# cure-lab/MotionCraft

Measured on AMD Instinct MI355X. Metric: sampled SMPL-X frames/sec (196-frame seq, 1000-step DDPM), higher is better.
Workload: dtype f32

## Files before the change

### include/motioncraft_amd.h

```cpp
#ifndef MOTIONCRAFT_AMD_H
#define MOTIONCRAFT_AMD_H
#include <stdint.h>

#ifdef __cplusplus
extern "C" {
#endif

#define MC_OK 0
#define MC_ERR_ARG 1
#define MC_ERR_HIP 2
#define MC_ERR_STATE 3

typedef struct mc_model mc_model;
typedef struct mc_ctx mc_ctx;

typedef struct mc_model_config {
    int32_t input_feats;
    int32_t max_seq_len;
    int32_t latent_dim;
    int32_t num_parts;
    int32_t num_layers;
    int32_t ffn_dim;
    int32_t time_embed_dim;
    int32_t text_latent_dim;
// ... 78 lines not shown

int mc_ctx_graph_capture(mc_ctx* c, float* x_dev, const float* noise_dev, const mc_step_coefs* coefs_host, int32_t num_steps,
                         void* stream);
int mc_ctx_graph_step(mc_ctx* c, int32_t step_index, void* stream);
int mc_ctx_graph_release(mc_ctx* c);

int mc_sample_step_seeded(mc_ctx* c, float* x_t_dev, int32_t step_index, const mc_step_coefs* coefs,
                          const float* noise_dev, const mc_seed* seed, float* x_prev_dev, float* x0_dev, void* stream);

int mc_sample_step_inpaint(mc_ctx* c, const float* x_t_dev, int32_t step_index, const mc_step_coefs* coefs,
                           const float* noise_dev, const mc_inpaint* inpaint, float* x_prev_dev, float* x0_dev,
                           void* stream);

int mc_ctx_get_buffer(mc_ctx* c, const char* name, int32_t layer, void** dev_ptr, int64_t* numel);

int mc_debug_flop_ledger(int32_t enable);
int64_t mc_debug_flop_ledger_dump(char* buf, int64_t cap);

int mc_op_gemm(const float* a_dev, const float* w_dev, const float* bias_dev, const float* res_dev,
               float* c_dev, int32_t M, int32_t N, int32_t K, int32_t ldw, int32_t act, void* stream);
int mc_op_gemm_f16(const float* a_dev, const float* w_dev, const float* bias_dev, const float* res_dev, float* c_dev,
                   int32_t M, int32_t N, int32_t K, int32_t split, void* stream);
int mc_op_gemm_f16_planes(const void* a_hi_dev, const void* a_lo_dev, const float* w_dev, const float* bias_dev, const float* res_dev,
                          float* c_dev, int32_t M, int32_t N, int32_t K, int32_t split, int32_t pre, int32_t frag_major, void* stream);
int mc_op_gemm_tail(const float* h_dev, const float* a_dev, const float* w_dev, const float* bias_dev, float* c_dev, float* c2_dev,
                    int32_t M, int32_t N, int32_t K, float wc, float wu, int32_t variant, void* stream);
int mc_op_ln_rows(const float* x_dev, int64_t ldx, const float* gamma_dev, const float* beta_dev,
                  const float* add_dev, int32_t add_mod, float* y_dev, int64_t rows, int32_t L, void* stream);
enum { MC_TEMPORAL_STEP = 0,
       MC_TEMPORAL_WHOLE = 1,
       MC_TEMPORAL_LSPLIT = 2,
       MC_TEMPORAL_PAIR = 3,
       MC_TEMPORAL_F16X3 = 4,
       MC_TEMPORAL_F16 = 5 };
int mc_op_body_attention(const float* mf_dev, int64_t ldmf, const float* qkv_dev, const float* wsm_dev, float* ys_dev, int64_t frames,
                         int32_t H, int32_t L, int64_t twin_from, const int32_t* split_flag_dev, int64_t frame0, void* stream);
int mc_op_temporal_attention(const float* mf_dev, const float* tf_dev, const float* mask_dev, float* yt_dev, int32_t b0, int32_t nb,
                             int32_t B, int32_t T, int32_t Nt, int32_t H, int32_t L, int32_t form, int32_t skip_text,
                             const int32_t* twin_flag_dev, void* stream);
enum { MC_ENC_ATTN_LAYER = 0,
       MC_ENC_ATTN_SMALL = 1,
       MC_ENC_ATTN_STREAM = 2 };
int mc_op_enc_ln(const float* x_dev, const float* gamma_dev, const float* beta_dev, float* y_dev, int64_t rows, int32_t L, float eps,
                 int32_t relu, void* stream);
int mc_op_enc_embed_tokens(const int32_t* ids_dev, const float* emb_dev, const float* pos_dev, float* x_dev, int64_t rows, int32_t S,
                           int32_t d, int32_t vocab, void* stream);
int mc_op_enc_attention(const float* qkv_dev, const uint8_t* valid_dev, float* out_dev, int32_t B, int32_t S, int32_t d, int32_t heads,
                        int32_t causal, int32_t form, void* stream);
typedef struct mc_gemm_strided {
    const float* a_dev; int64_t lda, a_gstride;
    const float* w_dev; int64_t ldw, w_gstride;
    const float* bias_dev; int64_t b_gstride;
    float* c_dev; int64_t ldc, c_gstride;
    const float* res_dev; int64_t ldr, r_gstride;
    const float* add_dev; int64_t ld_add, dup_rows;
    int32_t add_mod, act, act_after_res, M, N, K;
} mc_gemm_strided;
int mc_op_gemm_strided(int32_t mode, int32_t groups, const mc_gemm_strided* args, void* stream);
int mc_op_bigru_steps(const float* gi_dev, const float* whh_dev, const float* bhh_dev, float* h_dev, const int32_t* lens_dev,
                      int32_t len_div, int32_t B, int32_t S, int32_t H, int32_t s0, int32_t steps, void* stream);
int mc_op_conv1d_k4s2(const float* x_dev, int64_t ldx, const float* w_tapmajor_dev, const float* bias_dev, float* y_padded_dev, int32_t B,
                      int32_t T, int32_t C, int32_t Cp, int32_t O, float slope, void* stream);
int mc_op_sampler_update(const float* x_t_dev, const float* out_text_dev, const float* out_none_dev,
                         const float* noise_dev, float* x_prev_dev, float* x0_dev, int64_t n,
                         const mc_step_coefs* coefs, void* stream);

#define MC_POST_MAXTAP 129
// ... 187 lines not shown
```

### motioncraft_amd/csrc/mc_attn.hip

```cpp
#include "mc_common.h"
#include "mc_kernels.h"
#include <utility>
#include <stdlib.h>

namespace {

template <int HD, int H>
__global__ __launch_bounds__(256) void body_reg_k(const float* __restrict__ mf, long ldmf, const float* __restrict__ qkv,
                                                   const float* __restrict__ wsm, float* __restrict__ ys, long frames,
                                                   TwinAlias alias, long frame0) {
    constexpr int G = 8, L = G * HD;
    constexpr int GPW = 64 / HD;
    __shared__ float s_w[H * H];
    for (int i = threadIdx.x; i < H * H; i += 256) s_w[i] = wsm[i];
    __syncthreads();
    const int lane = threadIdx.x & 63;
    const long wave = (long)blockIdx.x * 4 + (threadIdx.x >> 6);
    const long grp = wave * GPW + lane / HD;
    const long frame = grp / G;
    const int gh = (int)(grp % G), l = lane % HD;
    if (frame >= frames) return;
    if (alias.split_flag && frame0 + frame >= alias.from && *alias.split_flag == 0) return;
    const int c = gh * HD + l;
    const long tok0 = frame * H;
// ... 35 lines not shown
        static_for_16(contract_kv);
#pragma unroll
        for (int h = 0; h < H; ++h) {
            float st = 0.f;
#pragma unroll
            for (int j = 0; j < H; ++j) st += s_w[h * H + j] * bv[j];
            float dy = 0.f;
            auto contract_qa = [&](auto S) { dy += row_ror<decltype(S)::value>(q[h]) * A_[decltype(S)::value]; };
            static_for_16(contract_qa);
            out[h * L] = st + (bv[h] + dy);
        }
    } else {
        float A[HD];
#pragma unroll
        for (int d = 0; d < HD; ++d) {
            float a = 0.f;
#pragma unroll
            for (int h = 0; h < H; ++h) a += __shfl(k[h], d, HD) * v[h];
            A[d] = a;
        }
#pragma unroll
        for (int h = 0; h < H; ++h) {
            float st = 0.f;
#pragma unroll
            for (int j = 0; j < H; ++j) st += s_w[h * H + j] * bv[j];
            float dy = 0.f;
#pragma unroll
            for (int d = 0; d < HD; ++d) dy += __shfl(q[h], d, HD) * A[d];
            out[h * L] = st + (bv[h] + dy);
        }
    }
}

template <int L, bool LSPLIT, bool PAIR = false>
__global__ __launch_bounds__(256, 3) void temporal_k(const float* __restrict__ mf, const float* __restrict__ tf,
                                                     const float* __restrict__ mask, float* __restrict__ yt,
                                                     int b0, int B, int T, int Nt, int H, const int* twin_flag, int skip_text) {
    static_assert(!PAIR || (L == 64 && !LSPLIT), "temporal_k: PAIR is the L = 64 whole-part form");
    constexpr int LW = PAIR ? 2 * L : L;
    constexpr int NT = L / 32;
    constexpr int LP = LW + 4;
    constexpr int C4 = LW / 4;
    constexpr int NSL = 256 / C4;
    constexpr int NACC = LSPLIT ? 1 : NT;
    __shared__ __attribute__((aligned(16))) float sm[2 * LW + 2 * NSL * LW + 2 * 32 * LP + (LSPLIT ? NT * 32 * 33 : 0)];
    float* s_m = sm;
    float* s_s = s_m + LW;
    float* s_pm = s_s + LW;
    float* s_ps = s_pm + NSL * LW;
    float* Ks = s_ps + NSL * LW;
    float* Vs = Ks + 32 * LP;
    float* Qs = Ks;
    float* Ps = Vs + 32 * LP;
    const int ls = LSPLIT ? (int)blockIdx.y : 0;

    const int tid = threadIdx.x, lane = tid & 63, wave = tid >> 6;
    const int HB = PAIR ? H / 2 : H;
    const int b = b0 + blockIdx.x / HB, h = PAIR ? 2 * (blockIdx.x % HB) : blockIdx.x % HB;
    const int wp = PAIR ? wave >> 1 : 0, wl = PAIR ? wave & 1 : wave;
    const float cnd = b < B ? 1.f : 0.f;
    const int bm = (twin_flag && b >= B && *twin_flag == 0) ? b - B : b;
    const float* mrow = mask + (long)(b % B) * T;
    const int Nseq = Nt + T;
    const float NEG = -1000000.f;
    const long D4 = 4 * L;
    const int hf = lane >> 5;

    auto row_ptr = [&](int n, int c4, int& t) -> const float* {
        const int nc = n < Nseq ? n : Nseq - 1;
        const bool txt = nc < Nt;
        t = txt ? 0 : nc - Nt;
        const int pp = PAIR ? c4 / L : 0, cc = PAIR ? c4 % L : c4;
        const float* rt = tf + ((long)b * Nt + (txt ? nc : 0)) * 2 * L + cc;
        const float* rm = mf + (((long)bm * T + t) * H + h + pp) * D4 + L + cc;
        return txt ? rt : rm;
    };
    auto issue_kv = [&](int n, int c4, f32x4& kk, f32x4& vv, float& mv) {
        int t;
        const float* r = row_ptr(n, c4, t);
        kk = *reinterpret_cast<const f32x4*>(r);
        vv = *reinterpret_cast<const f32x4*>(r + L);
        const float mm = mrow[t];
        mv = n < Nt ? cnd : mm;
    };
    auto issue_k = [&](int n, int c4, f32x4& kk, float& mv) {
        int t;
        const float* r = row_ptr(n, c4, t);
        kk = *reinterpret_cast<const f32x4*>(r);
        const float mm = mrow[t];
        mv = n < Nt ? cnd : mm;
    };

    constexpr int BATCH = LSPLIT ? 12 : 8;
    int skip1 = 0, skip2 = 0;
    if constexpr (!LSPLIT) {
        if (b >= B && skip_text) {
            int v = 0;
            for (int t = tid; t < T; t += 256) v |= mrow[t] != 0.f;
            if (__syncthreads_or(v)) { skip1 = Nt / (NSL * BATCH) * (NSL * BATCH); skip2 = Nt / 32 * 32; }
        }
    }

    {
        const int c4 = (tid % C4) * 4, sl = tid / C4;
        f32x4 m = {-3e38f, -3e38f, -3e38f, -3e38f}, s = {0.f, 0.f, 0.f, 0.f};
        for (int n0 = skip1 + sl; n0 < Nseq; n0 += NSL * BATCH) {
            f32x4 kk[BATCH];
            float mv[BATCH];
#pragma unroll
            for (int u = 0; u < BATCH; ++u) issue_k(n0 + u * NSL, c4, kk[u], mv[u]);
#pragma unroll
            for (int u = 0; u < BATCH; ++u) {
                const bool ok = n0 + u * NSL < Nseq;
                const float add = (1.f - mv[u]) * NEG;
#pragma unroll
                for (int j = 0; j < 4; ++j) kk[u][j] = ok ? (kk[u][j] + add) * LOG2E : -3e38f;
            }
#pragma unroll
            for (int j = 0; j < 4; ++j) {
                float nm = m[j];
#pragma unroll
                for (int u = 0; u < BATCH; ++u) nm = fmaxf(nm, kk[u][j]);
                float acc = s[j] * fast_exp2(m[j] - nm);
#pragma unroll
                for (int u = 0; u < BATCH; ++u) acc += fast_exp2(kk[u][j] - nm);
                s[j] = acc;
                m[j] = nm;
            }
        }
        *reinterpret_cast<f32x4*>(s_pm + sl * LW + c4) = m;
        *reinterpret_cast<f32x4*>(s_ps + sl * LW + c4) = s;
    }
    __syncthreads();
    if (tid < LW) {
        float M = -3e38f;
        for (int i = 0; i < NSL; ++i) M = fmaxf(M, s_pm[i * LW + tid]);
        float S = 0.f;
        for (int i = 0; i < NSL; ++i) S += s_ps[i * LW + tid] * fast_exp2(s_pm[i * LW + tid] - M);
        s_m[tid] = M;
        s_s[tid] = 1.f / S;
    }
    __syncthreads();

    const bool mm_active = PAIR || wave < NT;
    f32x16 acc[NACC];
#pragma unroll
    for (int dt = 0; dt < NACC; ++dt)
#pragma unroll
        for (int r = 0; r < 16; ++r) acc[dt][r] = 0.f;
    const int nch = (Nseq + 31) / 32;
    constexpr int SPT = (32 * C4) / 256;
    f32x4 pk[SPT], pv[SPT];
    float pm[SPT];
    auto prefetch_kv = [&](int ch) {
#pragma unroll
        for (int j = 0; j < SPT; ++j) {
            const int i = tid + 256 * j;
            issue_kv(ch * 32 + i / C4, (i % C4) * 4, pk[j], pv[j], pm[j]);
        }
    };
    const int ch0 = skip2 / 32;
    prefetch_kv(ch0);
    for (int ch = ch0; ch < nch; ++ch) {
#pragma unroll
        for (int j = 0; j < SPT; ++j) {
            const int i = tid + 256 * j;
            const int row = i / C4, c4 = (i % C4) * 4;
            const int n = ch * 32 + row;
            f32x4 e = {0.f, 0.f, 0.f, 0.f}, v = {0.f, 0.f, 0.f, 0.f};
            if (n < Nseq) {
                const float add = (1.f - pm[j]) * NEG;
#pragma unroll
                for (int q = 0; q < 4; ++q) {
                    e[q] = fast_exp2(fmaf(pk[j][q] + add, LOG2E, -s_m[c4 + q])) * s_s[c4 + q];
                    v[q] = pv[j][q] * pm[j];
                }
            }
            *reinterpret_cast<f32x4*>(Ks + row * LP + c4) = e;
            *reinterpret_cast<f32x4*>(Vs + row * LP + c4) = v;
        }
        __syncthreads();
        if (ch + 1 < nch) prefetch_kv(ch + 1);
        __builtin_amdgcn_sched_barrier(0);
        if (mm_active) {
#pragma unroll 4
            for (int ks = 0; ks < 16; ++ks) {
                const int n = 2 * ks + hf;
                if constexpr (LSPLIT) {
                    const float bb = Vs[n * LP + ls * 32 + (lane & 31)];
                    const float a = Ks[n * LP + wave * 32 + (lane & 31)];
                    acc[0] = __builtin_amdgcn_mfma_f32_32x32x2f32(a, bb, acc[0], 0, 0, 0);
                } else {
                    const float bb = Vs[n * LP + wp * L + wl * 32 + (lane & 31)];
#pragma unroll
                    for (int dt = 0; dt < NT; ++dt) {
                        const float a = Ks[n * LP + wp * L + dt * 32 + (lane & 31)];
                        acc[dt] = __builtin_amdgcn_mfma_f32_32x32x2f32(a, bb, acc[dt], 0, 0, 0);
                    }
                }
            }
        }
        __syncthreads();
    }

    const int ntc = (T + 31) / 32;
    constexpr int SEG = LW / 8;
    constexpr int QG = PAIR ? 4 : 8;
    const int qrow = tid >> 3, qsub = tid & 7;
    const int qpart = PAIR ? qsub >> 2 : 0, qcol = PAIR ? (qsub & 3) * SEG : qsub * SEG;
    float qv[SEG];
    auto prefetch_q = [&](int tc) {
        const int t = tc * 32 + qrow;
        if (t < T) {
            const float* r = mf + (((long)bm * T + t) * H + h + qpart) * D4 + 3 * L + qcol;
#pragma unroll
            for (int j = 0; j < SEG; j += 4) {
                const f32x4 x = *reinterpret_cast<const f32x4*>(r + j);
                qv[j] = x[0]; qv[j + 1] = x[1]; qv[j + 2] = x[2]; qv[j + 3] = x[3];
            }
        }
    };
    const int tc0 = LSPLIT ? (int)blockIdx.z : 0, tcs = LSPLIT ? (int)gridDim.z : 1;
    prefetch_q(tc0);
    for (int tc = tc0; tc < ntc; tc += tcs) {
        {
            const int t = tc * 32 + qrow;
            float mx = -3e38f;
            if (t < T) {
#pragma unroll
                for (int j = 0; j < SEG; ++j) mx = fmaxf(mx, qv[j]);
            }
            mx = group_max(mx, QG);
            float s = 0.f;
            if (t < T) {
#pragma unroll
// ... 46 lines not shown
            for (int i = tid; i < 32 * 32; i += 256) {
                const int tr = i >> 5, l = i & 31, t = tc * 32 + tr;
                float v = Ps[tr * 33 + l];
#pragma unroll
                for (int w = 1; w < NT; ++w) v += Ps[(w * 32 + tr) * 33 + l];
                if (t < T) yt[((long)b * T + t) * (H * L) + h * L + ls * 32 + l] = v;
            }
        }
    }
}

}

int mc_launch_body(const float* mf, long ldmf, const float* qkv, const float* wsm, float* ys,
                   long frames, int H, int L, int G, hipStream_t s, TwinAlias alias, long frame0) {
    MC_REQUIRE(G == 8 && (H == 12 || H == 8) && (L == 32 || L == 64 || L == 128), "body: H=%d L=%d G=%d unsupported", H, L, G);
    if (frames <= 0) return MC_OK;
    const int hd = L / G;
    const long groups = frames * G;
    const long waves = (groups * hd + 63) / 64;
    dim3 grid((unsigned)((waves + 3) / 4));
    MC_LEDGER("body_reg_k", grid, (double)frames * (2.0 * H * H * L + G * 2.0 * (2.0 * H * hd * hd)));
#define MC_BODY_CASE(HH)                                                                                          \
    if (hd == 16) hipLaunchKernelGGL((body_reg_k<16, HH>), grid, dim3(256), 0, s, mf, ldmf, qkv, wsm, ys, frames, alias, frame0);    \
    else if (hd == 8) hipLaunchKernelGGL((body_reg_k<8, HH>), grid, dim3(256), 0, s, mf, ldmf, qkv, wsm, ys, frames, alias, frame0); \
    else hipLaunchKernelGGL((body_reg_k<4, HH>), grid, dim3(256), 0, s, mf, ldmf, qkv, wsm, ys, frames, alias, frame0);
    if (H == 12) { MC_BODY_CASE(12) } else { MC_BODY_CASE(8) }
#undef MC_BODY_CASE
    MC_LAUNCH_CHECK();
    return MC_OK;
}

int mc_launch_temporal(const float* mf, const float* tf, const float* mask, float* yt,
                       int b0, int nb, int B, int T, int Nt, int H, int L, hipStream_t s, const int* twin_flag, long lsplit_max, bool pair, bool skip_text) {
    const int sk = skip_text ? 1 : 0;
    if (nb <= 0) return MC_OK;
    dim3 grid(nb * H), blk(256);
    if (mc_ledger_on) {
        char name[32];
        snprintf(name, sizeof(name), "temporal_k<%d", L);
        dim3 lg = grid;
        if (L >= 64 && (long)nb * H <= lsplit_max) { lg.y = L / 32; lg.z = (long)nb * H * (L / 32) * 2 <= 256 ? 2 : 1; }
        else if (L == 64 && pair && H % 2 == 0) lg.x = nb * (H / 2);
        MC_LEDGER(name, lg, (double)nb * H * (2.0 * (Nt + T) * L * L + 2.0 * T * L * L));
    }
    if (L >= 64 && (long)nb * H <= lsplit_max) {
        grid.y = L / 32;
        grid.z = (long)nb * H * (L / 32) * 2 <= 256 ? 2 : 1;
        if (L == 128) hipLaunchKernelGGL((temporal_k<128, true>), grid, blk, 0, s, mf, tf, mask, yt, b0, B, T, Nt, H, twin_flag, sk);
        else hipLaunchKernelGGL((temporal_k<64, true>), grid, blk, 0, s, mf, tf, mask, yt, b0, B, T, Nt, H, twin_flag, sk);
        MC_LAUNCH_CHECK();
        return MC_OK;
    }
    if (L == 128) hipLaunchKernelGGL((temporal_k<128, false>), grid, blk, 0, s, mf, tf, mask, yt, b0, B, T, Nt, H, twin_flag, sk);
    else if (L == 64 && pair && H % 2 == 0) {
        grid.x = nb * (H / 2);
        hipLaunchKernelGGL((temporal_k<64, false, true>), grid, blk, 0, s, mf, tf, mask, yt, b0, B, T, Nt, H, twin_flag, sk);
    } else if (L == 64) hipLaunchKernelGGL((temporal_k<64, false>), grid, blk, 0, s, mf, tf, mask, yt, b0, B, T, Nt, H, twin_flag, sk);
    else if (L == 32) hipLaunchKernelGGL((temporal_k<32, false>), grid, blk, 0, s, mf, tf, mask, yt, b0, B, T, Nt, H, twin_flag, sk);
    else { mc_set_error("temporal: latent_dim=%d unsupported (32, 64, 128)", L); return MC_ERR_ARG; }
    MC_LAUNCH_CHECK();
    return MC_OK;
}
```

### motioncraft_amd/csrc/mc_kernels.h

```cpp
#pragma once
#include <hip/hip_runtime.h>
#include <stdint.h>
#include "mc_options.h"

struct TwinAlias {
    const int* split_flag = nullptr;
    long from = 0;
};

int mc_launch_ln_rows(const float* X, long ldx, int x_col, const float* gamma, const float* beta,
                      const float* add, int add_mod, float* Y, long ldy, long rows, int L, hipStream_t s);
struct StepRef {
    const int* ptr = nullptr;
    long stride = 0;
};
int mc_launch_film_rows(const float* Y1, const float* Y2, const float* gamma, const float* beta,
                        const float* ss, float* A, long rows, int D, hipStream_t s, TwinAlias y1_alias = TwinAlias(), long row0 = 0,
                        StepRef step = StepRef(), int y1_parts = 1, long y1_pstride = 0,
                        int planes = 0, long plane_stride = 0);
int mc_launch_timestep_embedding(const int* t_orig, float* te, int S, int D, hipStream_t s);
int mc_launch_silu(const float* X, float* Y, long n, hipStream_t s);
int mc_launch_add_rows(float* out, const float* a, const float* b, const float* bias, long rows, int D, hipStream_t s);
int mc_launch_softmax_rows_small(const float* W, float* out, int rows, int cols, hipStream_t s);

// ... 56 lines not shown
    int* idx;
    float* gate;
    uint32_t* key;
    float* comb_w;
    int* src_row;
    int* dst_row;
    int* tile_group; int* tile_row0; int* tile_nrows;
    int* state;
    int max_tiles;
    uint32_t tie_xor = 0xFFFFFFFFu;
};
size_t mc_route_state_ints(int E);
bool mc_route_is_small(const McOptions& o, long N);
bool mc_route_cleans_counts(const McOptions& o, long N);
size_t mc_route_barrier_offset();
size_t mc_route_error_offset();
int mc_route_coop_wgs(long N);
int mc_route_coop_slots(int dev);
bool mc_route_coop_reserve(int dev, int nwg);
void mc_route_coop_release(int dev, int nwg);
size_t mc_route_barrier_ints();
int mc_launch_gate_finish(const float* proj, const float* sim_n, const float* logit_scale, long N, int E,
                          RouteBufs rb, hipStream_t s);
int mc_launch_route(long N, long Nsrc, long gsplit, int E, int capacity, RouteBufs rb, const McOptions& o, hipStream_t s);
const int* mc_route_num_tiles_ptr(const RouteBufs& rb, int group = 0);
const int* mc_route_split_flag_ptr(const RouteBufs& rb);

int mc_launch_body(const float* mf, long ldmf, const float* qkv, const float* wsm, float* ys,
                   long frames, int H, int L, int G, hipStream_t s, TwinAlias alias = TwinAlias(), long frame0 = 0);
int mc_launch_temporal(const float* mf, const float* tf, const float* mask, float* yt,
                       int b0, int nb, int B, int T, int Nt, int H, int L, hipStream_t s, const int* twin_flag = nullptr,
                       long lsplit_max = 96,
                       bool pair = false,
                       bool skip_text = false);
```

### motioncraft_amd/csrc/mc_model.hip

```cpp
#include "mc_ctx.h"

namespace {

template <class T>
int ws_alloc(mc_ctx* c, T** p, size_t n) {
    void* d = nullptr;
    size_t bytes = (n * sizeof(T) + 255) & ~(size_t)255;
    if (bytes == 0) bytes = 256;
    MC_HIP(hipMalloc(&d, bytes));
    c->allocs.push_back(d);
    c->bytes += (int64_t)bytes;
    *p = (T*)d;
    return MC_OK;
}

int bind_moe(const mc_model* m, const std::string& pre, int din, int dout, int seq_rows, MoeW* w) {
    const int64_t E = m->cfg.num_experts;
    w->din = din;
    w->dout = dout;
    return m->params.bind({{&w->emb, pre + "emb", (int64_t)seq_rows * din},       {&w->gate_w, pre + "gate_w", 256 * din},
                           {&w->gate_b, pre + "gate_b", 256},                      {&w->sim_n, pre + "sim_n", 256 * E},
                           {&w->sim_nT, pre + "sim_nT", 32 * 256},                 {&w->scale, pre + "scale", 1},
                           {&w->fc1_w, pre + "fc1_w", E * 4 * din * din},          {&w->fc1_b, pre + "fc1_b", E * 4 * din},
                           {&w->fc2_wt, pre + "fc2_wt", E * din * 4 * din},        {&w->fc2_b, pre + "fc2_b", E * din},
// ... 130 lines not shown

std::string check_chain(long v) {
    const long bad = v & ~kChainDefault;
    const int b = bad ? __builtin_ctzl((unsigned long)bad) : 0;
    return !bad ? "" : "chain bit " + std::to_string(b) + (b < kChainBits ? " is retired (DESIGN.md section 5)" : " is not defined");
}
std::string check_tune(long v) {
    const long bad = v & ~(long)kTuneBits;
    return !bad ? "" : v < 0 ? "gemm_tune: a bit mask (>= 0)" : "gemm_tune bit " + std::to_string(__builtin_ctzl(bad)) + " is not defined";
}
int chain_hook(mc_ctx* c, long& v) {
    const int L = c->m->cfg.latent_dim;
    c->hbuf_floats = ((v >> kChainMlp) & 1) && mc_mlp_supported(L, 4 * L) ? c->hbuf_cap : 0;
    return MC_OK;
}
int route_coop_hook(mc_ctx* c, long& v) {
    if (!v) {
        if (c->coop_reserved) { mc_route_coop_release(c->device, c->coop_reserved); c->coop_reserved = 0; }
    } else if (!c->opt.route_coop) {
        const int nwg = coop_grid_needed(c);
        MC_REQUIRE(nwg == 0 || mc_route_coop_reserve(c->device, nwg), "route_coop: the cooperative routing grid cannot be reserved on this device");
        c->coop_reserved = nwg;
        v = nwg > 0;
    }
    return MC_OK;
}

const OptionDef kOptions[] = {
    {"chain", "MC_CHAIN", nullptr, &McOptions::chain, kChainDefault, check_chain, chain_hook},
    {"small_gemm_rows", "MC_SMALL_GEMM_ROWS", nullptr, &McOptions::small_gemm_rows, 5600},
    {"split_rows_expert", "MC_SPLIT_ROWS_EXPERT", nullptr, &McOptions::split_rows_expert, 2048},
    {"split_rows_sffn", "MC_SPLIT_ROWS_SFFN", nullptr, &McOptions::split_rows_sffn, 8192},
    {"temporal_split", "MC_TEMPORAL_SPLIT", nullptr, &McOptions::temporal_split, 96},
    {"big_tokens", "MC_BIG_TOKENS", nullptr, &McOptions::big_tokens, 65536},
    {"rowchain_split", "MC_ROWCHAIN_SPLIT", nullptr, &McOptions::rowchain_split, 20480},
    {"gemm_tune", "MC_GEMM_TUNE", nullptr, &McOptions::gemm_tune, kTuneDefault, check_tune},
    {"small_tile_n", "MC_SMALL_TILE_N", nullptr, &McOptions::small_tile_n, 0,
     [](long v) -> std::string { return v == 0 || v == 48 || v == 64 || v == 96 ? "" : "small_tile_n: 0 (per-launch choice), 48, 64 or 96"; }},
    {"gemm_wp_grid", "MC_GEMM_WP_GRID", nullptr, &McOptions::gemm_wp_grid, 512},
    {"half_min_rows", "MC_HALF_MIN_ROWS", nullptr, &McOptions::half_min_rows, 512},
    {"gate_small", "MC_GATE_SMALL", nullptr, &McOptions::gate_small, 12000},
    {"split_expert", "MC_SPLIT_EXPERT", nullptr, &McOptions::split_expert, 0},
    {"split_sffn", "MC_SPLIT_SFFN", nullptr, &McOptions::split_sffn, 0},
    {"route_reg", "MC_ROUTE_REG", nullptr, &McOptions::route_reg, 1},
    {"route_coop", "MC_ROUTE_COOP", nullptr, &McOptions::route_coop, 1, nullptr, route_coop_hook},
    {"route_small", "MC_ROUTE_SMALL_CTX", "MC_ROUTE_SMALL", &McOptions::route_small, 20480,
     [](long v) -> std::string { return v >= 0 && v <= 131072 ? "" : "route_small: 0 .. 131072 pairs (the one-workgroup kernels hold at most 131072)"; }},
    {"route_per", nullptr, nullptr, &McOptions::route_per, 0,
     [](long v) -> std::string { return v == 0 || v == 10 || v == 16 ? "" : "route_per: 0 (default), 10 or 16"; }},
    {"dbg_delay_us", nullptr, nullptr, &McOptions::dbg_delay_us, 0,
     [](long v) -> std::string { return v >= -100000 && v <= 100000 ? "" : "dbg_delay_us: -100000 .. 100000"; }},
};

int seed_options(McOptions& o) {
    for (const OptionDef& d : kOptions) {
        const char *var = nullptr, *e = nullptr;
        for (const char* v : {d.env, d.env_alt})
            if (v && !e && (e = getenv(v))) var = v;
        const std::string why = e && d.check ? d.check(atol(e)) : "";
        MC_REQUIRE(why.empty(), "%s=%s: %s", var, e, why.c_str());
        o.*d.field = e ? atol(e) : d.dflt;
    }
    return MC_OK;
}

}
// ... 623 lines not shown
    MC_REQUIRE(variant != 2 || mc_gemm_tail_two_outputs(t),
               "gemm_tail variant 2: the block-range form is not eligible for M=%d N=%d K=%d (N <= 336, K %% 16 == 0, K >= 48, <= 17 blocks per wave)", M, N, K);
    int r = mc_launch_gemm_tail(t, (hipStream_t)stream);
    if (r == MC_OK && mc_gemm_tail_two_outputs(t))
        r = mc_launch_axpby(cdev, c2dev, 1.f, 1.f, cdev, (long)M * N, (hipStream_t)stream);
    return r;
}

int mc_op_ln_rows(const float* x, int64_t ldx, const float* gamma, const float* beta, const float* add, int32_t add_mod,
                  float* y, int64_t rows, int32_t L, void* stream) {
    return mc_launch_ln_rows(x, ldx, 0, gamma, beta, add, add_mod, y, L, rows, L, (hipStream_t)stream);
}

int mc_op_body_attention(const float* mf, int64_t ldmf, const float* qkv, const float* wsm, float* ys, int64_t frames, int32_t H, int32_t L,
                         int64_t twin_from, const int32_t* split_flag, int64_t frame0, void* stream) {
    MC_REQUIRE(mf && qkv && wsm && ys && frames >= 0 && ldmf >= L && twin_from >= 0 && frame0 >= 0, "bad body_attention args");
    TwinAlias alias;
    alias.split_flag = split_flag;
    alias.from = twin_from;
    return mc_launch_body(mf, ldmf, qkv, wsm, ys, frames, H, L, 8, (hipStream_t)stream, alias, frame0);
}

int mc_op_temporal_attention(const float* mf, const float* tf, const float* mask, float* yt, int32_t b0, int32_t nb, int32_t B, int32_t T,
                             int32_t Nt, int32_t H, int32_t L, int32_t form, int32_t skip_text, const int32_t* twin_flag, void* stream) {
    MC_REQUIRE(mf && tf && mask && yt && B > 0 && T > 0 && Nt > 0 && H > 0 && b0 >= 0 && nb >= 0 && b0 + nb <= 2 * B,
               "bad temporal_attention args");
    MC_REQUIRE(L == 32 || L == 64 || L == 128, "temporal_attention: latent_dim=%d unsupported (32, 64, 128)", L);
    hipStream_t s = (hipStream_t)stream;
    const bool sk = skip_text != 0;
    switch (form) {
    case MC_TEMPORAL_STEP: {
        const McOptions* o = mc_process_options();
        if (!o) return MC_ERR_ARG;
        return mc_launch_temporal(mf, tf, mask, yt, b0, nb, B, T, Nt, H, L, s, twin_flag, o->temporal_split, (o->chain >> kChainTemporalPair) & 1, sk);
    }
    case MC_TEMPORAL_WHOLE:
        return mc_launch_temporal(mf, tf, mask, yt, b0, nb, B, T, Nt, H, L, s, twin_flag, -1, false, sk);
    case MC_TEMPORAL_LSPLIT:
        MC_REQUIRE(L >= 64, "temporal_attention form LSPLIT: no column-sliced kernel at latent_dim=%d (64, 128)", L);
        return mc_launch_temporal(mf, tf, mask, yt, b0, nb, B, T, Nt, H, L, s, twin_flag, (long)nb * H, false, sk);
    case MC_TEMPORAL_PAIR:
        MC_REQUIRE(L == 64 && H % 2 == 0, "temporal_attention form PAIR: no two-part kernel at latent_dim=%d, num_parts=%d (64, even)", L, H);
        return mc_launch_temporal(mf, tf, mask, yt, b0, nb, B, T, Nt, H, L, s, twin_flag, -1, true, sk);
    case MC_TEMPORAL_F16X3:
    case MC_TEMPORAL_F16:
        MC_REQUIRE(L >= 64, "temporal_attention form %s: no fp16 kernel at latent_dim=%d (64, 128)", form == MC_TEMPORAL_F16X3 ? "F16X3" : "F16", L);
        return mc_launch_temporal_h(mf, tf, mask, yt, b0, nb, B, T, Nt, H, L, form == MC_TEMPORAL_F16X3, s, twin_flag, sk);
    }
    mc_set_error("temporal_attention: form %d (0 step, 1 WHOLE, 2 LSPLIT, 3 PAIR, 4 F16X3, 5 F16)", form);
    return MC_ERR_ARG;
}

int mc_op_sampler_update(const float* x_t, const float* ot, const float* on, const float* noise, float* x_prev, float* x0,
                         int64_t n, const mc_step_coefs* k, void* stream) {
    MC_REQUIRE(x_t && ot && on && noise && x_prev && k, "null argument");
    return mc_launch_sampler_update(x_t, ot, on, noise, x_prev, x0, n, to_coefs(k), (hipStream_t)stream);
}

}
```

### motioncraft_amd/csrc/mc_options.h

```cpp
#pragma once

enum ChainBit {
    kChainMlp = 0,
    kChainGate = 1,
    kChainRowchain = 2,
    kChainTwin = 4,
    kChainTwoStreams = 5,
    kChainGroupExperts = 6,
    kChainDeferTail = 7,
    kChainTwinAlias = 8,
    kChainCtrlGroups = 9,
    kChainProjQkv = 10,
    kChainTailGrouped = 11,
    kChainSffnPartials = 12,
    kChainDynSlices = 13,
    kChainSideBody = 14,
    kChainPqBody = 15,
    kChainTwinSplit = 16,
    kChainFilmPlanes = 17,
    kChainMlpDma = 18,
    kChainPadX = 19,
    kChainTemporalHalf = 20,
    kChainTailOnePass = 21,
    kChainTemporalPair = 22,
    kChainSkipText = 24,
    kChainStagger = 26,
    kChainResidualPre = 27,
    kChainFragMajor = 29,
    kChainBits = 30,
};
constexpr long kChainRetired = 1L << 3 | 1L << 23 | 1L << 25 | 1L << 28;
constexpr long kChainDefault = ((1L << kChainBits) - 1) & ~kChainRetired;
static_assert(kChainDefault == 763363319, "the default chain mask is public ABI");

struct McOptions {
    long chain, small_gemm_rows, split_rows_expert, split_rows_sffn, temporal_split, big_tokens, rowchain_split;
    long gemm_tune, small_tile_n, gemm_wp_grid, half_min_rows, gate_small, split_expert, split_sffn;
    long route_reg, route_coop, route_small, route_per, dbg_delay_us;
};

const McOptions* mc_process_options();
```

### motioncraft_amd/csrc/mc_step.hip

```cpp
#include "mc_ctx.h"

bool use_half(const mc_ctx* c) { return c->prec != MC_PREC_F32 && c->rows > c->opt.half_min_rows; }
static const HalfW* half_planes(const mc_ctx* c, const HalfW* hw) { return hw && hw->hi && use_half(c) ? hw : nullptr; }
static bool split3(const mc_ctx* c) { return c->prec == MC_PREC_F16X3; }

static bool twin_aliased(const mc_ctx* c, bool twin) { return twin && chain_on(c, kChainTwinAlias) && !c->no_alias; }
static TwinAlias twin_alias(const mc_ctx* c, bool twin, bool tokens) {
    return twin_aliased(c, twin) ? TwinAlias{mc_route_split_flag_ptr(c->rb), (tokens ? c->N : c->rows) / 2} : TwinAlias();
}

template <class Args>
static void set_tile_map(const mc_ctx* c, int group, Args& a) {
    const long to = (long)group * c->rb.max_tiles;
    a.tile_group = c->rb.tile_group + to; a.tile_row0 = c->rb.tile_row0 + to; a.tile_nrows = c->rb.tile_nrows + to;
    a.num_tiles = mc_route_num_tiles_ptr(c->rb, group);
}

static int dbg_hold(const mc_ctx* c, hipStream_t pos, hipStream_t neg) {
    const long us = c->opt.dbg_delay_us;
    return us == 0 ? MC_OK : mc_launch_spin((us > 0 ? us : -us) * 100, us > 0 ? pos : neg);
}

int dense(const mc_ctx* c, const float* A, long lda, const float* W, long ldw, const float* bias, const float* R, long ldr,
          float* C, long ldc, long M, int N, int K, int act, hipStream_t s) {
// ... 205 lines not shown
static int layer_body(mc_ctx* c, int i, bool twin, long row0, long nrows, hipStream_t sb) {
    const mc_model_config& g = c->m->cfg;
    const int L = g.latent_dim, H = g.num_parts, D = L * H;
    const LayerW& w = c->lw[i];
    const long tok0 = row0 * H, ntok = nrows * H;
    int r;
    if (pq_fused(c)) {
    } else if (chain_on(c, kChainRowchain) && mc_mlp_supported(L, 32)) {
        RowChainArgs q;
        q.split_tokens = c->opt.rowchain_split;
        q.X = c->mf; q.ldx = 4 * L; q.gamma = w.dyn_g; q.beta = w.dyn_b; q.W = w.qkv_w; q.bias = w.qkv_b;
        q.Y = c->qkv; q.ldy = 3 * L; q.tok0 = tok0; q.N = tok0 + ntok; q.L = L; q.Nout = 3 * L;
        q.alias = twin_alias(c, twin, true);
        if ((r = mc_launch_rowchain(1, q, sb))) return r;
    } else {
        if ((r = mc_launch_ln_rows(c->mf + tok0 * 4 * L, 4 * L, 0, w.dyn_g, w.dyn_b, nullptr, 1, c->z + tok0 * L, L, ntok, L, sb))) return r;
        if ((r = dense(c, c->z + tok0 * L, L, w.qkv_w, L, w.qkv_b, nullptr, 0, c->qkv + tok0 * 3 * L, 3 * L, ntok, 3 * L, L, ACT_NONE, sb))) return r;
    }
    if (body_fused(c)) return MC_OK;
    return mc_launch_body(c->mf + tok0 * 4 * L, 4 * L, c->qkv + tok0 * 3 * L, w.wsm, c->ys + row0 * D, nrows, H, L, g.dyn_heads, sb,
                          twin_alias(c, twin, false), row0);
}

static int layer_temporal(mc_ctx* c, int i, bool twin, long row0, long nrows, hipStream_t stt) {
    const mc_model_config& g = c->m->cfg;
    const int L = g.latent_dim, H = g.num_parts;
    const float* tfl = c->tf + (long)i * c->Ntxt * 2 * L;
    const int* twin_flag = twin_alias(c, twin, true).split_flag;
    const int tnb = (int)(nrows / c->T);
    if (use_half(c) && chain_on(c, kChainTemporalHalf) && (L == 128 || L == 64) && (long)tnb * H > c->opt.temporal_split)
        return mc_launch_temporal_h(c->mf, tfl, c->mask, c->yt, (int)(row0 / c->T), tnb, c->B, c->T, g.max_text_len, H, L,
                                    split3(c), stt, twin_flag, chain_on(c, kChainSkipText));
    return mc_launch_temporal(c->mf, tfl, c->mask, c->yt, (int)(row0 / c->T), tnb, c->B, c->T,
                              g.max_text_len, H, L, stt, twin_flag, c->opt.temporal_split, chain_on(c, kChainTemporalPair), chain_on(c, kChainSkipText));
}

static int layer_rows(mc_ctx* c, int i, bool twin, long row0, long nrows, hipStream_t s, hipStream_t st) {
    int r;
    if ((r = layer_proj(c, i, twin, row0, nrows, s))) return r;
    hipStream_t sb = s, stt = s;
    if (st != s) {
        MC_HIP(hipEventRecord(c->ev_fork, s));
        MC_HIP(hipStreamWaitEvent(st, c->ev_fork, 0));
        if (chain_on(c, kChainSideBody) && c->rows <= 1200) sb = st; else stt = st;
        if ((r = dbg_hold(c, st, s))) return r;
    }
    if ((r = layer_body(c, i, twin, row0, nrows, sb))) return r;
    if (sb != s) MC_HIP(hipEventRecord(c->ev_join, sb));
    if ((r = layer_temporal(c, i, twin, row0, nrows, stt))) return r;
    if (stt != s) MC_HIP(hipEventRecord(c->ev_join, stt));
    if (st != s) MC_HIP(hipStreamWaitEvent(s, c->ev_join, 0));
    return MC_OK;
}

static int layer_rows_tail(mc_ctx* c, int i, float* hs, int step, bool twin, long row0, long nrows, hipStream_t s, hipEvent_t ev_rows = nullptr,
                           hipEvent_t wait_first = nullptr) {
    if (wait_first) MC_HIP(hipStreamWaitEvent(s, wait_first, 0));
    const mc_model_config& g = c->m->cfg;
    const int L = g.latent_dim, H = g.num_parts, D = L * H, F = g.ffn_dim;
    const LayerW& w = c->lw[i];
    int r;
    const float* ss0 = c->ss + ((long)(i * 2 + 0) * c->maxS + step) * 2 * D;
    if ((r = film_block(c, hs, c->ys, c->yt, w.ca_ln_g, w.ca_ln_b, ss0, w.ca_out_w, w.ca_out_b, row0, nrows, s, false, twin_alias(c, twin, false), &w.h_ca_out, 1,
                        ev_rows))) return r;
    const long o = row0 * D;
    int z2_parts = 1;
    if (chain_on(c, kChainMlp) && mc_mlp_supported(L, F)) {
// ... 329 lines not shown
```

### motioncraft_amd/lib.py

```python
import ctypes
import os

import numpy as np

_HERE = os.path.dirname(os.path.abspath(__file__))
LIB_PATH = os.path.join(_HERE, 'libmotioncraft_amd.so')

MC_OK = 0
ACT_NONE, ACT_GELU, ACT_SILU = 0, 1, 2
TEMPORAL_FORMS = dict(step=0, whole=1, lsplit=2, pair=3, f16x3=4, f16=5)


class ModelConfig(ctypes.Structure):
    _fields_ = [(n, ctypes.c_int32) for n in (
        'input_feats', 'max_seq_len', 'latent_dim', 'num_parts', 'num_layers', 'ffn_dim',
        'time_embed_dim', 'text_latent_dim', 'max_text_len', 'num_experts', 'topk', 'dyn_heads')] + [
        ('capacity_factor', ctypes.c_float), ('cfg_scale', ctypes.c_float),
        ('num_ctrl_layers', ctypes.c_int32), ('ctrl_cond_feats', ctypes.c_int32), ('ctrl_condition_cfg', ctypes.c_int32)]


class StepCoefs(ctypes.Structure):
    _fields_ = [('mode', ctypes.c_int32)] + [(n, ctypes.c_float) for n in (
        'text_coef', 'none_coef', 'c1', 'c2', 'log_var', 'sqrt_recip', 'sqrt_recipm1', 'ab', 'ab_prev',
        'eta', 'nonzero')]


_P = ctypes.c_void_p
ENC_ATTN_FORMS = dict(layer=0, small=1, stream=2)
GM_PLAIN, GM_ENC = 0, 4


class GemmStrided(ctypes.Structure):
    _fields_ = [('a_dev', _P), ('lda', ctypes.c_int64), ('a_gstride', ctypes.c_int64),
                ('w_dev', _P), ('ldw', ctypes.c_int64), ('w_gstride', ctypes.c_int64),
                ('bias_dev', _P), ('b_gstride', ctypes.c_int64),
                ('c_dev', _P), ('ldc', ctypes.c_int64), ('c_gstride', ctypes.c_int64),
                ('res_dev', _P), ('ldr', ctypes.c_int64), ('r_gstride', ctypes.c_int64),
                ('add_dev', _P), ('ld_add', ctypes.c_int64), ('dup_rows', ctypes.c_int64)] + [
        (n, ctypes.c_int32) for n in ('add_mod', 'act', 'act_after_res', 'M', 'N', 'K')]


class Inpaint(ctypes.Structure):
    _fields_ = [('gt_dev', ctypes.c_void_p), ('keep_dev', ctypes.c_void_p), ('gt_noise_dev', ctypes.c_void_p),
# ... 228 lines not shown
```

Before: 662.8.

## Fuse temporal attention softmax statistics into a single online pass over keys

Adds a one-pass variant of the temporal attention kernel. It tracks a running column max and sum per chunk and rescales the MFMA accumulators, replacing the separate max/sum pre-pass over all keys. The one-pass form is on by default for latent_dim >= 64 and can be turned off with an option; the old two-pass forms stay available as explicit forms. This avoids re-reading K and a full extra loop, at the cost of a per-chunk accumulator rescale and an extra barrier and shared-memory reduction per chunk.

```diff
diff --git a/include/motioncraft_amd.h b/include/motioncraft_amd.h
--- a/include/motioncraft_amd.h
+++ b/include/motioncraft_amd.h
@@ -134,7 +134,9 @@
        MC_TEMPORAL_LSPLIT = 2,
        MC_TEMPORAL_PAIR = 3,
        MC_TEMPORAL_F16X3 = 4,
-       MC_TEMPORAL_F16 = 5 };
+       MC_TEMPORAL_F16 = 5,
+       MC_TEMPORAL_WHOLE_2PASS = 6,
+       MC_TEMPORAL_PAIR_2PASS = 7 };
 int mc_op_body_attention(const float* mf_dev, int64_t ldmf, const float* qkv_dev, const float* wsm_dev, float* ys_dev, int64_t frames,
                          int32_t H, int32_t L, int64_t twin_from, const int32_t* split_flag_dev, int64_t frame0, void* stream);
 int mc_op_temporal_attention(const float* mf_dev, const float* tf_dev, const float* mask_dev, float* yt_dev, int32_t b0, int32_t nb,
diff --git a/motioncraft_amd/csrc/mc_attn.hip b/motioncraft_amd/csrc/mc_attn.hip
--- a/motioncraft_amd/csrc/mc_attn.hip
+++ b/motioncraft_amd/csrc/mc_attn.hip
@@ -91,17 +91,19 @@
     }
 }
 
-template <int L, bool LSPLIT, bool PAIR = false>
+template <int L, bool LSPLIT, bool PAIR = false, bool ONEPASS = false>
 __global__ __launch_bounds__(256, 3) void temporal_k(const float* __restrict__ mf, const float* __restrict__ tf,
                                                      const float* __restrict__ mask, float* __restrict__ yt,
                                                      int b0, int B, int T, int Nt, int H, const int* twin_flag, int skip_text) {
     static_assert(!PAIR || (L == 64 && !LSPLIT), "temporal_k: PAIR is the L = 64 whole-part form");
+    static_assert(!ONEPASS || !LSPLIT, "temporal_k: the column-sliced form keeps its two passes");
     constexpr int LW = PAIR ? 2 * L : L;
     constexpr int NT = L / 32;
     constexpr int LP = LW + 4;
     constexpr int C4 = LW / 4;
     constexpr int NSL = 256 / C4;
     constexpr int NACC = LSPLIT ? 1 : NT;
+    static_assert(256 % C4 == 0, "temporal_k: every staging thread keeps one float4 column");
     __shared__ __attribute__((aligned(16))) float sm[2 * LW + 2 * NSL * LW + 2 * 32 * LP + (LSPLIT ? NT * 32 * 33 : 0)];
     float* s_m = sm;
     float* s_s = s_m + LW;
@@ -160,7 +162,7 @@
         }
     }
 
-    {
+    if constexpr (!ONEPASS) {
         const int c4 = (tid % C4) * 4, sl = tid / C4;
         f32x4 m = {-3e38f, -3e38f, -3e38f, -3e38f}, s = {0.f, 0.f, 0.f, 0.f};
         for (int n0 = skip1 + sl; n0 < Nseq; n0 += NSL * BATCH) {
@@ -189,17 +191,17 @@
         }
         *reinterpret_cast<f32x4*>(s_pm + sl * LW + c4) = m;
         *reinterpret_cast<f32x4*>(s_ps + sl * LW + c4) = s;
-    }
-    __syncthreads();
-    if (tid < LW) {
-        float M = -3e38f;
-        for (int i = 0; i < NSL; ++i) M = fmaxf(M, s_pm[i * LW + tid]);
-        float S = 0.f;
-        for (int i = 0; i < NSL; ++i) S += s_ps[i * LW + tid] * fast_exp2(s_pm[i * LW + tid] - M);
-        s_m[tid] = M;
-        s_s[tid] = 1.f / S;
-    }
-    __syncthreads();
+        __syncthreads();
+        if (tid < LW) {
+            float M = -3e38f;
+            for (int i = 0; i < NSL; ++i) M = fmaxf(M, s_pm[i * LW + tid]);
+            float S = 0.f;
+            for (int i = 0; i < NSL; ++i) S += s_ps[i * LW + tid] * fast_exp2(s_pm[i * LW + tid] - M);
+            s_m[tid] = M;
+            s_s[tid] = 1.f / S;
+        }
+        __syncthreads();
+    }
 
     const bool mm_active = PAIR || wave < NT;
     f32x16 acc[NACC];
@@ -220,36 +222,76 @@
     };
     const int ch0 = skip2 / 32;
     prefetch_kv(ch0);
-    for (int ch = ch0; ch < nch; ++ch) {
-#pragma unroll
-        for (int j = 0; j < SPT; ++j) {
-            const int i = tid + 256 * j;
-            const int row = i / C4, c4 = (i % C4) * 4;
-            const int n = ch * 32 + row;
-            f32x4 e = {0.f, 0.f, 0.f, 0.f}, v = {0.f, 0.f, 0.f, 0.f};
-            if (n < Nseq) {
+    if constexpr (ONEPASS) {
+        const int c4 = (tid % C4) * 4, sl = tid / C4;
+        float* s_f = s_m;
+        f32x4 m = {-3e38f, -3e38f, -3e38f, -3e38f}, s = {0.f, 0.f, 0.f, 0.f};
+        auto chunk_max = [&](int ch) {
+            f32x4 cm = {-3e38f, -3e38f, -3e38f, -3e38f};
+#pragma unroll
+            for (int j = 0; j < SPT; ++j) {
+                const bool ok = ch * 32 + sl + NSL * j < Nseq;
                 const float add = (1.f - pm[j]) * NEG;
 #pragma unroll
                 for (int q = 0; q < 4; ++q) {
-                    e[q] = fast_exp2(fmaf(pk[j][q] + add, LOG2E, -s_m[c4 + q])) * s_s[c4 + q];
-                    v[q] = pv[j][q] * pm[j];
-                }
-            }
-            *reinterpret_cast<f32x4*>(Ks + row * LP + c4) = e;
-            *reinterpret_cast<f32x4*>(Vs + row * LP + c4) = v;
-        }
-        __syncthreads();
-        if (ch + 1 < nch) prefetch_kv(ch + 1);
-        __builtin_amdgcn_sched_barrier(0);
-        if (mm_active) {
+                    pk[j][q] = ok ? (pk[j][q] + add) * LOG2E : -3e38f;
+                    cm[q] = fmaxf(cm[q], pk[j][q]);
+                }
+            }
+            *reinterpret_cast<f32x4*>(s_pm + sl * LW + c4) = cm;
+        };
+        chunk_max(ch0);
+        __syncthreads();
+        for (int ch = ch0; ch < nch; ++ch) {
+            f32x4 f, add = {0.f, 0.f, 0.f, 0.f};
+            {
+                f32x4 cm = *reinterpret_cast<const f32x4*>(s_pm + c4);
+#pragma unroll
+                for (int i = 1; i < NSL; ++i) {
+                    const f32x4 x = *reinterpret_cast<const f32x4*>(s_pm + i * LW + c4);
+#pragma unroll
+                    for (int q = 0; q < 4; ++q) cm[q] = fmaxf(cm[q], x[q]);
+                }
+#pragma unroll
+                for (int q = 0; q < 4; ++q) {
+                    const float nm = fmaxf(m[q], cm[q]);
+                    f[q] = fast_exp2(m[q] - nm);
+                    m[q] = nm;
+                }
+            }
+#pragma unroll
+            for (int j = 0; j < SPT; ++j) {
+                const int row = sl + NSL * j;
+                const bool ok = ch * 32 + row < Nseq;
+                f32x4 e, v;
+#pragma unroll
+                for (int q = 0; q < 4; ++q) {
+                    e[q] = fast_exp2(pk[j][q] - m[q]);
+                    add[q] += e[q];
+                    v[q] = ok ? pv[j][q] * pm[j] : 0.f;
+                }
+                *reinterpret_cast<f32x4*>(Ks + row * LP + c4) = e;
+                *reinterpret_cast<f32x4*>(Vs + row * LP + c4) = v;
+            }
+#pragma unroll
+            for (int q = 0; q < 4; ++q) s[q] = fmaf(s[q], f[q], add[q]);
+            if (sl == 0) *reinterpret_cast<f32x4*>(s_f + c4) = f;
+            __syncthreads();
+            if (ch + 1 < nch) prefetch_kv(ch + 1);
+            __builtin_amdgcn_sched_barrier(0);
+            if (mm_active) {
+                const float* fp = s_f + wp * L + 4 * hf;
+#pragma unroll
+                for (int dt = 0; dt < NT; ++dt)
+#pragma unroll
+                    for (int q = 0; q < 4; ++q) {
+                        const f32x4 ff = *reinterpret_cast<const f32x4*>(fp + dt * 32 + 8 * q);
+#pragma unroll
+                        for (int i = 0; i < 4; ++i) acc[dt][4 * q + i] *= ff[i];
+                    }
 #pragma unroll 4
-            for (int ks = 0; ks < 16; ++ks) {
-                const int n = 2 * ks + hf;
-                if constexpr (LSPLIT) {
-                    const float bb = Vs[n * LP + ls * 32 + (lane & 31)];
-                    const float a = Ks[n * LP + wave * 32 + (lane & 31)];
-                    acc[0] = __builtin_amdgcn_mfma_f32_32x32x2f32(a, bb, acc[0], 0, 0, 0);
-                } else {
+                for (int ks = 0; ks < 16; ++ks) {
+                    const int n = 2 * ks + hf;
                     const float bb = Vs[n * LP + wp * L + wl * 32 + (lane & 31)];
 #pragma unroll
                     for (int dt = 0; dt < NT; ++dt) {
@@ -258,8 +300,71 @@
                     }
                 }
             }
-        }
-        __syncthreads();
+            __builtin_amdgcn_sched_barrier(0);
+            if (ch + 1 < nch) chunk_max(ch + 1);
+            __syncthreads();
+        }
+        *reinterpret_cast<f32x4*>(s_ps + sl * LW + c4) = s;
+        __syncthreads();
+        if (tid < LW) {
+            float S = 0.f;
+            for (int i = 0; i < NSL; ++i) S += s_ps[i * LW + tid];
+            s_s[tid] = 1.f / S;
+        }
+        __syncthreads();
+        if (mm_active) {
+            const float* sp = s_s + wp * L + 4 * hf;
+#pragma unroll
+            for (int dt = 0; dt < NT; ++dt)
+#pragma unroll
+                for (int q = 0; q < 4; ++q) {
+                    const f32x4 ff = *reinterpret_cast<const f32x4*>(sp + dt * 32 + 8 * q);
+#pragma unroll
+                    for (int i = 0; i < 4; ++i) acc[dt][4 * q + i] *= ff[i];
+                }
+        }
+    } else {
+        for (int ch = ch0; ch < nch; ++ch) {
+#pragma unroll
+            for (int j = 0; j < SPT; ++j) {
+                const int i = tid + 256 * j;
+                const int row = i / C4, c4 = (i % C4) * 4;
+                const int n = ch * 32 + row;
+                f32x4 e = {0.f, 0.f, 0.f, 0.f}, v = {0.f, 0.f, 0.f, 0.f};
+                if (n < Nseq) {
+                    const float add = (1.f - pm[j]) * NEG;
+#pragma unroll
+                    for (int q = 0; q < 4; ++q) {
+                        e[q] = fast_exp2(fmaf(pk[j][q] + add, LOG2E, -s_m[c4 + q])) * s_s[c4 + q];
+                        v[q] = pv[j][q] * pm[j];
+                    }
+                }
+                *reinterpret_cast<f32x4*>(Ks + row * LP + c4) = e;
+                *reinterpret_cast<f32x4*>(Vs + row * LP + c4) = v;
+            }
+            __syncthreads();
+            if (ch + 1 < nch) prefetch_kv(ch + 1);
+            __builtin_amdgcn_sched_barrier(0);
+            if (mm_active) {
+#pragma unroll 4
+                for (int ks = 0; ks < 16; ++ks) {
+                    const int n = 2 * ks + hf;
+                    if constexpr (LSPLIT) {
+                        const float bb = Vs[n * LP + ls * 32 + (lane & 31)];
+                        const float a = Ks[n * LP + wave * 32 + (lane & 31)];
+                        acc[0] = __builtin_amdgcn_mfma_f32_32x32x2f32(a, bb, acc[0], 0, 0, 0);
+                    } else {
+                        const float bb = Vs[n * LP + wp * L + wl * 32 + (lane & 31)];
+#pragma unroll
+                        for (int dt = 0; dt < NT; ++dt) {
+                            const float a = Ks[n * LP + wp * L + dt * 32 + (lane & 31)];
+                            acc[dt] = __builtin_amdgcn_mfma_f32_32x32x2f32(a, bb, acc[dt], 0, 0, 0);
+                        }
+                    }
+                }
+            }
+            __syncthreads();
+        }
     }
 
     const int ntc = (T + 31) / 32;
@@ -372,7 +477,8 @@
 }
 
 int mc_launch_temporal(const float* mf, const float* tf, const float* mask, float* yt,
-                       int b0, int nb, int B, int T, int Nt, int H, int L, hipStream_t s, const int* twin_flag, long lsplit_max, bool pair, bool skip_text) {
+                       int b0, int nb, int B, int T, int Nt, int H, int L, hipStream_t s, const int* twin_flag, long lsplit_max, bool pair, bool skip_text,
+                       bool onepass) {
     const int sk = skip_text ? 1 : 0;
     if (nb <= 0) return MC_OK;
     dim3 grid(nb * H), blk(256);
@@ -392,13 +498,19 @@
         MC_LAUNCH_CHECK();
         return MC_OK;
     }
-    if (L == 128) hipLaunchKernelGGL((temporal_k<128, false>), grid, blk, 0, s, mf, tf, mask, yt, b0, B, T, Nt, H, twin_flag, sk);
+#define MC_TEMPORAL_CASE(LL, PP)                                                                                                              \
+    do {                                                                                                                                       \
+        if (onepass) hipLaunchKernelGGL((temporal_k<LL, false, PP, true>), grid, blk, 0, s, mf, tf, mask, yt, b0, B, T, Nt, H, twin_flag, sk);  \
+        else hipLaunchKernelGGL((temporal_k<LL, false, PP, false>), grid, blk, 0, s, mf, tf, mask, yt, b0, B, T, Nt, H, twin_flag, sk);         \
+    } while (0)
+    if (L == 128) MC_TEMPORAL_CASE(128, false);
     else if (L == 64 && pair && H % 2 == 0) {
         grid.x = nb * (H / 2);
-        hipLaunchKernelGGL((temporal_k<64, false, true>), grid, blk, 0, s, mf, tf, mask, yt, b0, B, T, Nt, H, twin_flag, sk);
-    } else if (L == 64) hipLaunchKernelGGL((temporal_k<64, false>), grid, blk, 0, s, mf, tf, mask, yt, b0, B, T, Nt, H, twin_flag, sk);
-    else if (L == 32) hipLaunchKernelGGL((temporal_k<32, false>), grid, blk, 0, s, mf, tf, mask, yt, b0, B, T, Nt, H, twin_flag, sk);
+        MC_TEMPORAL_CASE(64, true);
+    } else if (L == 64) MC_TEMPORAL_CASE(64, false);
+    else if (L == 32) MC_TEMPORAL_CASE(32, false);
     else { mc_set_error("temporal: latent_dim=%d unsupported (32, 64, 128)", L); return MC_ERR_ARG; }
+#undef MC_TEMPORAL_CASE
     MC_LAUNCH_CHECK();
     return MC_OK;
 }
diff --git a/motioncraft_amd/csrc/mc_kernels.h b/motioncraft_amd/csrc/mc_kernels.h
--- a/motioncraft_amd/csrc/mc_kernels.h
+++ b/motioncraft_amd/csrc/mc_kernels.h
@@ -112,4 +112,6 @@
                        int b0, int nb, int B, int T, int Nt, int H, int L, hipStream_t s, const int* twin_flag = nullptr,
                        long lsplit_max = 96,
                        bool pair = false,
-                       bool skip_text = false);
+                       bool skip_text = false,
+                       bool onepass = false);
+inline bool mc_temporal_step_onepass(long option, int L) { return option != 0 && L >= 64; }
diff --git a/motioncraft_amd/csrc/mc_model.hip b/motioncraft_amd/csrc/mc_model.hip
--- a/motioncraft_amd/csrc/mc_model.hip
+++ b/motioncraft_amd/csrc/mc_model.hip
@@ -186,6 +186,8 @@
     {"split_rows_expert", "MC_SPLIT_ROWS_EXPERT", nullptr, &McOptions::split_rows_expert, 2048},
     {"split_rows_sffn", "MC_SPLIT_ROWS_SFFN", nullptr, &McOptions::split_rows_sffn, 8192},
     {"temporal_split", "MC_TEMPORAL_SPLIT", nullptr, &McOptions::temporal_split, 96},
+    {"temporal_onepass", "MC_TEMPORAL_ONEPASS", nullptr, &McOptions::temporal_onepass, 1,
+     [](long v) -> std::string { return v == 0 || v == 1 ? "" : "temporal_onepass: 0 (two passes over the keys) or 1 (one)"; }},
     {"big_tokens", "MC_BIG_TOKENS", nullptr, &McOptions::big_tokens, 65536},
     {"rowchain_split", "MC_ROWCHAIN_SPLIT", nullptr, &McOptions::rowchain_split, 20480},
     {"gemm_tune", "MC_GEMM_TUNE", nullptr, &McOptions::gemm_tune, kTuneDefault, check_tune},
@@ -875,22 +877,25 @@
     case MC_TEMPORAL_STEP: {
         const McOptions* o = mc_process_options();
         if (!o) return MC_ERR_ARG;
-        return mc_launch_temporal(mf, tf, mask, yt, b0, nb, B, T, Nt, H, L, s, twin_flag, o->temporal_split, (o->chain >> kChainTemporalPair) & 1, sk);
+        return mc_launch_temporal(mf, tf, mask, yt, b0, nb, B, T, Nt, H, L, s, twin_flag, o->temporal_split, (o->chain >> kChainTemporalPair) & 1, sk,
+                                  mc_temporal_step_onepass(o->temporal_onepass, L));
     }
     case MC_TEMPORAL_WHOLE:
-        return mc_launch_temporal(mf, tf, mask, yt, b0, nb, B, T, Nt, H, L, s, twin_flag, -1, false, sk);
+    case MC_TEMPORAL_WHOLE_2PASS:
+        return mc_launch_temporal(mf, tf, mask, yt, b0, nb, B, T, Nt, H, L, s, twin_flag, -1, false, sk, form == MC_TEMPORAL_WHOLE);
     case MC_TEMPORAL_LSPLIT:
         MC_REQUIRE(L >= 64, "temporal_attention form LSPLIT: no column-sliced kernel at latent_dim=%d (64, 128)", L);
         return mc_launch_temporal(mf, tf, mask, yt, b0, nb, B, T, Nt, H, L, s, twin_flag, (long)nb * H, false, sk);
     case MC_TEMPORAL_PAIR:
+    case MC_TEMPORAL_PAIR_2PASS:
         MC_REQUIRE(L == 64 && H % 2 == 0, "temporal_attention form PAIR: no two-part kernel at latent_dim=%d, num_parts=%d (64, even)", L, H);
-        return mc_launch_temporal(mf, tf, mask, yt, b0, nb, B, T, Nt, H, L, s, twin_flag, -1, true, sk);
+        return mc_launch_temporal(mf, tf, mask, yt, b0, nb, B, T, Nt, H, L, s, twin_flag, -1, true, sk, form == MC_TEMPORAL_PAIR);
     case MC_TEMPORAL_F16X3:
     case MC_TEMPORAL_F16:
         MC_REQUIRE(L >= 64, "temporal_attention form %s: no fp16 kernel at latent_dim=%d (64, 128)", form == MC_TEMPORAL_F16X3 ? "F16X3" : "F16", L);
         return mc_launch_temporal_h(mf, tf, mask, yt, b0, nb, B, T, Nt, H, L, form == MC_TEMPORAL_F16X3, s, twin_flag, sk);
     }
-    mc_set_error("temporal_attention: form %d (0 step, 1 WHOLE, 2 LSPLIT, 3 PAIR, 4 F16X3, 5 F16)", form);
+    mc_set_error("temporal_attention: form %d (0 step, 1 WHOLE, 2 LSPLIT, 3 PAIR, 4 F16X3, 5 F16, 6 WHOLE_2PASS, 7 PAIR_2PASS)", form);
     return MC_ERR_ARG;
 }
 
diff --git a/motioncraft_amd/csrc/mc_options.h b/motioncraft_amd/csrc/mc_options.h
--- a/motioncraft_amd/csrc/mc_options.h
+++ b/motioncraft_amd/csrc/mc_options.h
@@ -36,7 +36,7 @@
 struct McOptions {
     long chain, small_gemm_rows, split_rows_expert, split_rows_sffn, temporal_split, big_tokens, rowchain_split;
     long gemm_tune, small_tile_n, gemm_wp_grid, half_min_rows, gate_small, split_expert, split_sffn;
-    long route_reg, route_coop, route_small, route_per, dbg_delay_us;
+    long route_reg, route_coop, route_small, route_per, dbg_delay_us, temporal_onepass;
 };
 
 const McOptions* mc_process_options();
diff --git a/motioncraft_amd/csrc/mc_step.hip b/motioncraft_amd/csrc/mc_step.hip
--- a/motioncraft_amd/csrc/mc_step.hip
+++ b/motioncraft_amd/csrc/mc_step.hip
@@ -261,7 +261,8 @@
         return mc_launch_temporal_h(c->mf, tfl, c->mask, c->yt, (int)(row0 / c->T), tnb, c->B, c->T, g.max_text_len, H, L,
                                     split3(c), stt, twin_flag, chain_on(c, kChainSkipText));
     return mc_launch_temporal(c->mf, tfl, c->mask, c->yt, (int)(row0 / c->T), tnb, c->B, c->T,
-                              g.max_text_len, H, L, stt, twin_flag, c->opt.temporal_split, chain_on(c, kChainTemporalPair), chain_on(c, kChainSkipText));
+                              g.max_text_len, H, L, stt, twin_flag, c->opt.temporal_split, chain_on(c, kChainTemporalPair), chain_on(c, kChainSkipText),
+                              mc_temporal_step_onepass(c->opt.temporal_onepass, L));
 }
 
 static int layer_rows(mc_ctx* c, int i, bool twin, long row0, long nrows, hipStream_t s, hipStream_t st) {
diff --git a/motioncraft_amd/lib.py b/motioncraft_amd/lib.py
--- a/motioncraft_amd/lib.py
+++ b/motioncraft_amd/lib.py
@@ -8,7 +8,7 @@
 
 MC_OK = 0
 ACT_NONE, ACT_GELU, ACT_SILU = 0, 1, 2
-TEMPORAL_FORMS = dict(step=0, whole=1, lsplit=2, pair=3, f16x3=4, f16=5)
+TEMPORAL_FORMS = dict(step=0, whole=1, lsplit=2, pair=3, f16x3=4, f16=5, whole_2pass=6, pair_2pass=7)
 
 
 class ModelConfig(ctypes.Structure):
```

Measured after the change: 665.6 (median of 6 runs). No clear change (+0.4%).
